# JasperSnoek/spearmint

Measured on AMD Instinct MI355X. Metric: EI candidate evaluations per second (N_cand x mcmc_iters / wall time), higher is better.
Workload: dtype f64; 1 GPU; C3: synthetic 32D, N_obs=2048, 200k candidates/GPU, mcmc_iters=20; N_obs=2048, candidates_per_gpu=200000, D=32, mcmc_iters=20, collective=torch.distributed all_gather_into_tensor

## Files before the change

### spearmint_amd/csrc/common.h

```cpp
#pragma once
#include <hip/hip_runtime.h>
#include <stdint.h>

typedef double d4 __attribute__((ext_vector_type(4)));
typedef double d2 __attribute__((ext_vector_type(2)));

#define MFMA_F64(a, b, c) __builtin_amdgcn_mfma_f64_16x16x4f64((a), (b), (c), 0, 0, 0)

#define SPX_NB 64
#define SPX_BM 128
#define SPX_BN 128
#define SPX_BK 16
#define SPX_PADN 128

#define SPX_COV_MATERN52 0
#define SPX_COV_MATERN32 1
#define SPX_COV_ARDSE 2

#define SPX_HT 4

static inline int64_t round_up(int64_t x, int64_t m) { return (x + m - 1) / m * m; }

void spx_note_attr_error(const char* kernel, size_t lds_bytes, hipError_t e);
#define SPX_LDS_ATTR(fn, bytes)                                                                                            \
    do {                                                                                                                   \
        hipError_t ae_ = hipFuncSetAttribute(reinterpret_cast<const void*>(fn), hipFuncAttributeMaxDynamicSharedMemorySize, \
                                             (int)(bytes));                                                                \
        if (ae_ != hipSuccess) spx_note_attr_error(#fn, (size_t)(bytes), ae_);                                             \
    } while (0)

void launch_scale_rows(hipStream_t s, const double* x, int64_t n, int64_t n_pad, int D, int Dp,
                       const double* ls , int ls_stride, int nh, double factor,
                       double* xs , double* sumsq ,
                       double* xs2 = nullptr ,
                       int* zero_ints = nullptr , int n_zero = 0);
void launch_lean_prologue(hipStream_t s, const double* x, int64_t n, int64_t n_pad, int D, int Dp, const double* ls,
                          int ls_stride, int nh, double* xs, double* sumsq, double* xs2, const double* vals,
                          const double* htab, double* rhs, int* info, int* flags, int64_t vals_stride = 0);
void launch_cov_self(hipStream_t s, const double* Xs, const double* s1, const double* X2s,
                     const double* htab, double* K, int N, int Np, int Dp, int nh, bool tiled = false,
                     int kind = SPX_COV_MATERN52);
void launch_cov_cross(hipStream_t s, const double* Xs, const double* s1, const double* Cs,
                      const double* s2, const double* htab, double* Kst, int N, int Np, int Mc,
                      int Dp, int nh, int kind = SPX_COV_MATERN52, int live_rows = 0 ,
                      bool allow_flat = true );
void launch_cross_mean(hipStream_t s, const double* Xs, const double* s1, const double* Cs,
                       const double* s2, const double* htab, const double* alpha, double* out,
                       int N, int Np, int Mc, int Dp, int nh, int kind = SPX_COV_MATERN52);
void launch_constraint_prob(hipStream_t s, const double* Xs, const double* s1, const double* Cs,
                            const double* s2, const double* htab, const double* alpha, double* out,
                            int N, int Np, int Mc, int Dp, int nh, int kind);
void launch_constraint_const(hipStream_t s, const double* htab, double* out, int Mc, int nh);

void launch_chol_diag(hipStream_t s, double* L, double* Dinv, int* info, int Np, int k, int nh, int updated = 0);
void launch_chol_panel(hipStream_t s, double* L, const double* Dinv, int Np, int k, int nh, double* rhs = nullptr);
void launch_lean_step(hipStream_t s, double* Lt, double* Dinv, int* info, double* rhs, double* diagL, int Np, int k,
                      int nh, int lazy);
void launch_lean_trsm(hipStream_t s, double* Lt, const double* Dinv, double* rhs, int Np, int k, int nh);
void launch_lean_step_ps(hipStream_t s, double* Lt, double* Dinv, int* info, double* rhs, double* diagL, int* flags,
                         int Np, int k, int nh);
struct FlowFused {
    const double* comp; const double* hyp; const double* vals; int D, hs;
    double* lp_out; int* info_out;
    int64_t vals_stride;
};
void launch_lean_flow(hipStream_t s, double* Lt, double* Dinv, int* info, double* rhs, double* diagL, int* lflags,
                      int* dflags, unsigned* tickets, int Np, int nh, int gen, bool alone,
                      const double* Xs, const double* X2s, const double* s1, const double* htab, int N, int Dp, int kind,
                      int* cu_busy, int spin_limit = 0, const FlowFused* fused = nullptr);
void launch_lean_rhs_init(hipStream_t s, const double* vals, const double* htab, double* rhs, int N, int Np, int nh,
                          int* info, int* flags, int64_t vals_stride = 0);
void launch_lean_logprob(hipStream_t s, const double* diagL, const double* rhs, const int* info, double* out, int* info_out,
                         int N, int Np, int nh);
void launch_trinv(hipStream_t s, const double* L, const double* Dinv, double* WT, int Np, int nh, bool tiled = false);
void launch_gamma(hipStream_t s, const double* WT, const double* vals, const double* htab,
                  double* gamma, int N, int Np, int nh);
void launch_gamma_multi(hipStream_t s, const double* WT_h, const double* rhs, const double* htab_h,
                        double* gamma, int N, int Np, int S);
// ... 57 lines not shown
```

### spearmint_amd/csrc/cov_kernels.hip

```cpp
#include "common.h"
#include "ei_device.h"

#ifndef SPX_COV_HOIST
#define SPX_COV_HOIST 1
#endif

#define SR_DC 32
template <int ROWS>
__device__ __forceinline__ void scale_rows_body(
    const double* __restrict__ x, int64_t n, int64_t n_pad, int D, int Dp,
    const double* __restrict__ ls, int ls_stride, double factor,
    double* __restrict__ xs, double* __restrict__ sumsq, double* __restrict__ xs2, int bx, int h)
{
#pragma clang fp contract(off)
    __shared__ double T[ROWS][SR_DC + 1];
    const int tid = threadIdx.x;
    const int64_t row0 = (int64_t)bx * ROWS;
    const int rows = (int)((n_pad - row0 < ROWS) ? (n_pad - row0) : ROWS);
    const int64_t row = row0 + tid;
    const double* lsh = ls + (size_t)h * ls_stride;
    double* o = xs + ((size_t)h * n_pad + row0) * Dp;
    double* o2 = xs2 ? xs2 + ((size_t)h * n_pad + row0) * Dp : nullptr;
    double acc = 0.0;
    for (int d0 = 0; d0 < Dp; d0 += SR_DC) {
// ... 246 lines not shown
    const double* __restrict__ Cs, const double* __restrict__ s2,
    const double* __restrict__ htab, const double* __restrict__ alpha,
    double* __restrict__ out, int N, int Np, int Mc, int Dp, int nchunks, int64_t ldo, int rows_per_wg, int live_rows)
{
    const int jtop = (MODE == 0 && live_rows > 0) ? live_rows : Np;
    const int jbeg = (MODE == 2 || MODE == 4) ? 0 : blockIdx.y * rows_per_wg;
    const int jend = (MODE == 2 || MODE == 4) ? Np : min(jtop, jbeg + rows_per_wg);
    cov_run<MODE, QC, KIND>(Xs, s1, Cs, s2, htab, alpha, out, N, Np, Mc, Dp, nchunks, ldo, blockIdx.z, blockIdx.x * 64, jbeg, jend);
}

template <int QC, int KIND>
__global__ __launch_bounds__(256, 2) void k_cov_flat(
    const double* __restrict__ Xs, const double* __restrict__ s1,
    const double* __restrict__ Cs, const double* __restrict__ s2,
    const double* __restrict__ htab, double* __restrict__ out, int N, int Np, int Mc, int Dp, int nchunks, int64_t ldo, int nh,
    int live_rows)
{
    const int jtop = live_rows > 0 ? live_rows : Np;
    const int nrc = (jtop + 127) >> 7, ncb = Mc >> 6;
    const int64_t per_h = (int64_t)ncb * nrc, U = per_h * nh;
    int64_t u = U * blockIdx.x / gridDim.x;
    const int64_t u1 = U * (blockIdx.x + 1) / gridDim.x;
    while (u < u1) {
        const int h = (int)(u / per_h);
        const int rem = (int)(u - (int64_t)h * per_h);
        const int cb = rem / nrc, rc = rem - cb * nrc;
        const int run = (int)min((int64_t)(nrc - rc), u1 - u);
        cov_run<0, QC, KIND>(Xs, s1, Cs, s2, htab, nullptr, out, N, Np, Mc, Dp, nchunks, ldo, h, cb * 64, rc * 128,
                             min(jtop, (rc + run) * 128));
        u += run;
    }
}

template <int MODE, int KIND>
static void launch_cov_kind(hipStream_t s, const double* Xs, const double* s1, const double* Cs,
                            const double* s2, const double* htab, const double* alpha, double* out,
                            int N, int Np, int Mc, int Dp, int nh, int64_t ldo, int live_rows, bool allow_flat)
{
    const int Q = Dp / 4;
    int rows_per_wg = (Np >= 1024) ? 512 : ((Np >= 256) ? 256 : 128);
#ifdef SPX_DEV_KNOBS
    static const char* rpw = getenv("SPX_COV_RPW");
    if (rpw && MODE == 3) rows_per_wg = atoi(rpw);
#endif
    const int row_top = (MODE == 0 && live_rows > 0) ? live_rows : Np;
    dim3 grid(Mc / 64, (MODE == 2 || MODE == 4) ? 1 : (row_top + rows_per_wg - 1) / rows_per_wg, nh);
    dim3 block(256);
    if (MODE == 0) {
        const int64_t places = 2 * (int64_t)spx_cov_cus(), wgs = (int64_t)grid.x * grid.y * grid.z;
        const int64_t units = (int64_t)nh * (Mc / 64) * (((live_rows > 0 ? live_rows : Np) + 127) / 128);
        if (wgs > places && units >= 4 * places && allow_flat) {
            const int64_t rounds = (units + 16 * places - 1) / (16 * places);
            const dim3 fgrid((unsigned)(places * rounds));
#define SPX_COVF_LAUNCH(QC_)                                                                                   \
    hipLaunchKernelGGL((k_cov_flat<QC_, KIND>), fgrid, block, 0, s, Xs, s1, Cs, s2, htab, out, N, Np, Mc, Dp, Q / QC_, ldo, nh, live_rows)
            if (Q == 1) SPX_COVF_LAUNCH(1);
            else if (Q == 2) SPX_COVF_LAUNCH(2);
            else if (Q == 4) SPX_COVF_LAUNCH(4);
            else SPX_COVF_LAUNCH(8);
#undef SPX_COVF_LAUNCH
            return;
        }
    }
#define SPX_COV_LAUNCH(QC_)                                                                        \
    hipLaunchKernelGGL((k_cov<MODE, QC_, KIND>), grid, block, 0, s, Xs, s1, Cs, s2, htab, alpha, out, N, \
                       Np, Mc, Dp, Q / QC_, ldo, rows_per_wg, live_rows)
// ... 60 lines not shown
```

### spearmint_amd/csrc/predict_kernels.hip

```cpp
#include "common.h"
#include "np_sum.h"
#include "ei_device.h"

#define BM SPX_BM
#define BN SPX_BN
#define BK SPX_BK
#define LDT 144

template <int NW, int STG, int ABL>
__global__ __launch_bounds__(64 * NW, NW / 2) void k_predict_gemm(
    const double* __restrict__ WT, const double* __restrict__ Kst,
    const double* __restrict__ gamma, double* __restrict__ part_ss,
    double* __restrict__ part_bg, int Np, int Mc, int nh, int ncb, int nrb,
    int part_nh , int part_h0 ,
    const double* __restrict__ gammaS , int S,
    double* __restrict__ part_bgS )
{
    extern __shared__ __attribute__((aligned(16))) double smem[];
    double* As = smem;
    double* Bs = smem + 2 * BK * LDT;

    const int tid = threadIdx.x;
    const int lane = tid & 63, wave = tid >> 6;
    const int g = lane >> 4, li = lane & 15;
// ... 241 lines not shown
    const int h = rem / ncbx;
    const int cb = (rem % ncbx) * 8 + xcd;
    if (cb >= ncb) return;

    const double* Ag = WT + (size_t)h * Np * Np + (size_t)ib * BM;
    const double* Bg = Kst + (size_t)h * Np * Mc + (size_t)cb * BN;
    const int nk = (ib + 1) * (BM / BK);
    typedef __attribute__((address_space(3))) void lds_void_t;
    const unsigned loff = (unsigned)lane * 16u;
    d4 acc[4][4];
#pragma unroll
    for (int mt = 0; mt < 4; ++mt)
#pragma unroll
        for (int nt = 0; nt < 4; ++nt) acc[mt][nt] = (d4){0.0, 0.0, 0.0, 0.0};

#define SPX_DMA_ROW(GPTR_, LPTR_)                                                                          \
    asm volatile("s_mov_b32 m0, %2\n\ts_nop 0\n\tglobal_load_lds_dwordx4 %0, %1"                          \
                 :: "v"(loff), "s"(GPTR_), "s"((unsigned)(size_t)(lds_void_t*)(LPTR_)) : "memory")
#define SPX_DMA_TILE(KT_, BUF_)                                                                            \
    {                                                                                                      \
        const size_t j0_ = (size_t)(KT_) * BK;                                                             \
        _Pragma("unroll") for (int q = 0; q < NQ; ++q) {                                                   \
            const int row = wave + NW * q;                                                                 \
            SPX_DMA_ROW(Ag + (j0_ + row) * Np, As + (BUF_) * BK * LDT + row * LDT);                        \
            SPX_DMA_ROW(Bg + (j0_ + row) * Mc, Bs + (BUF_) * BK * LDT + row * LDT);                        \
        }                                                                                                  \
    }
    SPX_DMA_TILE(0, 0)
    asm volatile("s_waitcnt vmcnt(0)" ::: "memory");
    __syncthreads();

    const int nfull = nk - BM / BK;
    int cur = 0;
    for (int j = 0; j < nk; ++j) {
        const int m0 = (j >= nfull) ? ((j - nfull - wm + 1) >> 1) : 0;
        if (j + 1 < nk) SPX_DMA_TILE(j + 1, cur ^ 1)
        const double* Ac = As + cur * BK * LDT + 16 * wm + li;
        const double* Bc = Bs + cur * BK * LDT + 64 * wn + li;
        if (m0 == 0) {
#pragma unroll
            for (int k0 = 0; k0 < BK; k0 += 4) {
                double a[4], b[4];
#pragma unroll
                for (int t = 0; t < 4; ++t) b[t] = Bc[(k0 + g) * LDT + 16 * t];
#pragma unroll
                for (int t = 0; t < 4; ++t) a[t] = Ac[(k0 + g) * LDT + 32 * t];
#pragma unroll
                for (int mt = 0; mt < 4; ++mt)
#pragma unroll
                    for (int nt = 0; nt < 4; ++nt) acc[mt][nt] = MFMA_F64(a[mt], b[nt], acc[mt][nt]);
            }
            asm volatile("s_waitcnt vmcnt(0)" ::: "memory");
            __syncthreads();
        } else {
#define SPX_TRI_G4(MT_)                                                      \
    _Pragma("unroll") for (int nt = 0; nt < 4; ++nt) acc[MT_][nt] = MFMA_F64(a[MT_], b[nt], acc[MT_][nt]);
#pragma unroll
            for (int k0 = 0; k0 < BK; k0 += 4) {
                double a[4], b[4];
#pragma unroll
                for (int t = 0; t < 4; ++t) b[t] = Bc[(k0 + g) * LDT + 16 * t];
#pragma unroll
                for (int t = 0; t < 4; ++t) a[t] = Ac[(k0 + g) * LDT + 32 * t];
                switch (m0) {
                    case 1: SPX_TRI_G4(1)
                    case 2: SPX_TRI_G4(2)
                    case 3: SPX_TRI_G4(3)
                    default: break;
                }
            }
#undef SPX_TRI_G4
            asm volatile("s_waitcnt vmcnt(0)" ::: "memory");
            __syncthreads();
        }
        cur ^= 1;
    }
#undef SPX_DMA_TILE
#undef SPX_DMA_ROW

    const double* gh = gamma + (size_t)h * Np + (size_t)ib * BM + 16 * wm;
    double gam[4][4];
#pragma unroll
    for (int mt = 0; mt < 4; ++mt)
#pragma unroll
        for (int r = 0; r < 4; ++r) gam[mt][r] = gh[32 * mt + g + 4 * r];
    double* red = smem;
#pragma unroll
    for (int nt = 0; nt < 4; ++nt) {
        double ss = 0.0, bg = 0.0;
#pragma unroll
        for (int mt = 0; mt < 4; ++mt)
#pragma unroll
            for (int r = 0; r < 4; ++r) {
                const double v = acc[mt][nt][r];
                ss = fma(v, v, ss);
                bg = fma(v, gam[mt][r], bg);
            }
        ss += __shfl_xor(ss, 16);
        bg += __shfl_xor(bg, 16);
        ss += __shfl_xor(ss, 32);
        bg += __shfl_xor(bg, 32);
        if (g == 0) {
            const int c = 64 * wn + 16 * nt + li;
            red[(wm * BN + c) * 2 + 0] = ss;
            red[(wm * BN + c) * 2 + 1] = bg;
        }
    }
// ... 500 lines not shown
```

### spearmint_amd/csrc/spx_api.hip

```cpp
#include <math.h>
#include <stdarg.h>
#include <stdio.h>
#include <string.h>

#include <algorithm>
#include <string>
#include <vector>

#include <chrono>

#include "spx_internal.h"
#include "np_sum.h"

#define SPX_VERSION 200

static const char* kStageNames[ST_COUNT] = {
    "scale_rows", "cov_self", "chol_diag", "chol_panel", "trinv", "gamma_alpha",
    "cov_cross", "cross_mean", "predict_gemm", "ei_finalize", "mean_argmax",
    "factor_total", "ei_run_total"};


std::string& spx_err_slot()
{
    static thread_local std::string g_err;
// ... 6 lines not shown
    return g_attr;
}

void spx_note_attr_error(const char* kernel, size_t lds_bytes, hipError_t e)
{
    char buf[384];
    snprintf(buf, sizeof buf, "hipFuncSetAttribute(%s, MaxDynamicSharedMemorySize = %zu) failed: %s", kernel, lds_bytes,
             hipGetErrorString(e));
    (void)hipGetLastError();
    if (spx_attr_err_slot().empty()) spx_attr_err_slot() = buf;
}

int spx_fail(int code, const char* fmt, ...)
{
    char buf[512];
    va_list ap;
    va_start(ap, fmt);
    vsnprintf(buf, sizeof buf, fmt, ap);
    va_end(ap);
    spx_err_slot() = buf;
    if (!spx_attr_err_slot().empty()) {
        spx_err_slot() += " [also: " + spx_attr_err_slot() + "]";
        spx_attr_err_slot().clear();
    }
    return code;
}

static int ensure_init(spx_handle* h)
{
    HIPCHK(hipSetDevice(h->device));
    if (!h->inited) {
        HIPCHK(hipStreamCreateWithFlags(&h->stream, hipStreamNonBlocking));
        HIPCHK(hipStreamCreateWithFlags(&h->stream2, hipStreamNonBlocking));
        for (int i = 0; i < 6; ++i) HIPCHK(hipEventCreateWithFlags(&h->ev_sync[i], hipEventDisableTiming));
        HIPCHK(hipEventCreate(&h->ev_t0));
        HIPCHK(hipEventCreate(&h->ev_t1));
        HIPCHK(hipEventCreateWithFlags(&h->ev_obs, hipEventDisableTiming));
        HIPCHK(hipEventCreateWithFlags(&h->ev_p0, hipEventDisableTiming));
        HIPCHK(hipEventCreateWithFlags(&h->ev_fac, hipEventDisableTiming));
        int ncu = 0;
        if (hipDeviceGetAttribute(&ncu, hipDeviceAttributeMultiprocessorCount, h->device) == hipSuccess && ncu > 0) h->n_cu = ncu;
        h->inited = true;
    }
    return SPX_OK;
}

static int ev_begin(spx_handle* h, int stage, hipStream_t strm)
{
    if (!h->timing) return -1;
    if (h->ev_used == h->ev_pool.size()) {
        spx_handle::Ev e;
        if (hipEventCreate(&e.a) != hipSuccess || hipEventCreate(&e.b) != hipSuccess) return -1;
        h->ev_pool.push_back(e);
    }
    spx_handle::Ev& e = h->ev_pool[h->ev_used];
    e.stage = stage;
    (void)hipEventRecord(e.a, strm);
    return (int)h->ev_used++;
}
static void ev_end(spx_handle* h, int id, hipStream_t strm)
{
    if (id >= 0) (void)hipEventRecord(h->ev_pool[id].b, strm);
}
static void ev_collect(spx_handle* h)
{
    for (size_t i = 0; i < h->ev_used; ++i) {
// ... 28 lines not shown
extern "C" {

int spx_version(void) { return SPX_VERSION; }
const char* spx_last_error(void) { return spx_err_slot().c_str(); }

int spx_device_count(void)
{
    int n = 0;
    hipError_t e = hipGetDeviceCount(&n);
    if (e != hipSuccess) return fail(SPX_ERR_HIP, "hipGetDeviceCount: %s", hipGetErrorString(e));
    return n;
}

int spx_create(int device_id, spx_handle** out)
{
    if (!out || device_id < 0) return fail(SPX_ERR_ARG, "spx_create: bad arguments");
    spx_handle* h = new spx_handle();
    h->device = device_id;
    *out = h;
    return SPX_OK;
}

void spx_destroy(spx_handle* h)
{
    if (!h) return;
    if (h->multi) { spx_multi_destroy(h->multi); delete h; return; }
    spx_comm_release(h);
    if (h->con) { spx_destroy(h->con); h->con = nullptr; }
    if (h->full) { spx_destroy(h->full); h->full = nullptr; }
    if (h->inited) {
        (void)hipSetDevice(h->device);
        (void)hipStreamSynchronize(h->stream);
        (void)hipStreamSynchronize(h->stream2);
        DevBuf* bufs[] = {&h->comp, &h->vals, &h->ldur, &h->cand, &h->hyp, &h->htab, &h->Xs, &h->X2s,
                          &h->s1, &h->Lm, &h->WT, &h->Dinv, &h->gamma, &h->alpha, &h->info, &h->lp,
                          &h->Cs[0], &h->s2[0], &h->Kst[0], &h->part_ss[0], &h->part_bg[0], &h->time_m[0],
                          &h->Cs[1], &h->s2[1], &h->Kst[1], &h->part_ss[1], &h->part_bg[1], &h->time_m[1],
                          &h->fantT, &h->gammaS, &h->bests, &h->part_bgS[0], &h->part_bgS[1],
                          &h->pt_x, &h->pt_k, &h->pt_dk, &h->pt_t, &h->pt_z, &h->pt_out, &h->pt_kt, &h->pt_dkt,
                          &h->ei_draw, &h->ei_mean, &h->mom_m, &h->mom_v, &h->mom_t, &h->am_val, &h->am_idx,
                          &h->am_out_val, &h->am_out_idx, &h->scratch, &h->sobol_dirs, &h->sobol_out, &h->rhs, &h->diagL, &h->ps_flags, &h->flow_flags,
                          &h->alphaS, &h->pt_u, &h->rec_send, &h->rec_recv, &h->rec_out, &h->ei_sum_full,
                          &h->con_tab, &h->con_Cs[0], &h->con_Cs[1], &h->con_s2[0], &h->con_s2[1], &h->con_p[0], &h->con_p[1],
                          &h->mom_c, &h->rhs_rows};
        for (DevBuf* b : bufs) b->release();
        h->pin_up.release();
        h->pin_res.release();
        h->pin_stage.release();
        for (auto& e : h->ev_pool) { (void)hipEventDestroy(e.a); (void)hipEventDestroy(e.b); }
        for (int i = 0; i < 6; ++i) (void)hipEventDestroy(h->ev_sync[i]);
        (void)hipEventDestroy(h->ev_t0);
        (void)hipEventDestroy(h->ev_t1);
        (void)hipEventDestroy(h->ev_obs);
        (void)hipEventDestroy(h->ev_p0);
        (void)hipEventDestroy(h->ev_fac);
        (void)hipStreamDestroy(h->stream);
        (void)hipStreamDestroy(h->stream2);
    }
    delete h;
}

int spx_set_option(spx_handle* h, const char* name, int64_t value)
{
    if (!h || !name) return fail(SPX_ERR_ARG, "spx_set_option: null");
    if (h->multi) return spx_multi_set_option(h->multi, name, value);
    if (!strcmp(name, "kstar_budget_bytes")) {
        h->kst_budget = value > 0 ? value : (512ll << 20);
        return SPX_OK;
    }
    if (!strcmp(name, "gemm_waves")) {
        if (!predict_gemm_variant_ok((int)value))
            return fail(SPX_ERR_ARG, "spx_set_option: gemm_waves=%lld is not a variant of this build", (long long)value);
        h->gemm_variant = (int)value;
        return SPX_OK;
    }
    if (!strcmp(name, "covar")) {
        if (value < SPX_COVAR_MATERN52 || value > SPX_COVAR_SE)
            return fail(SPX_ERR_ARG, "spx_set_option: covar=%lld is not one of SPX_COVAR_*", (long long)value);
        if (h->cov_kind != (int)value) { h->factored = false; h->ran = false; h->ran_time = false; h->S = 0; h->full_valid = false; }
        h->cov_kind = (int)value;
        return SPX_OK;
    }
    if (!strcmp(name, "lean_lazy")) {
        h->lean_lazy = value < 0 ? -1 : (value != 0);
        return SPX_OK;
    }
    if (!strcmp(name, "step_overlap")) {
        h->step_overlap = value < 0 ? -1 : (value != 0);
        return SPX_OK;
    }
// ... 21 lines not shown
        h->lean_flow = value < 0 ? -1 : (value != 0);
        h->flow_demoted = false;
        h->flow_clean = 0;
        return SPX_OK;
    }
    if (!strcmp(name, "flow_rearm_after")) {
        h->flow_rearm_after = value < 0 ? 16 : (int)std::min<int64_t>(value, 1 << 30);
        return SPX_OK;
    }
    if (!strcmp(name, "flow_spin_limit")) {
        h->flow_spin_limit = value <= 0 ? 0 : (int)std::min<int64_t>(value, 1 << 30);
        return SPX_OK;
    }
    if (!strcmp(name, "lean_ps")) {
        h->lean_ps = value < 0 ? -1 : (value != 0);
        return SPX_OK;
    }
    if (!strcmp(name, "lean_merge")) {
        h->lean_merge = value < 0 ? -1 : (value != 0);
        return SPX_OK;
    }
    if (!strcmp(name, "lean_one")) {
        h->lean_one = value < 0 ? -1 : (value != 0);
        return SPX_OK;
    }
    if (!strcmp(name, "lean_poll")) { h->lean_poll = value < 0 ? -1 : (value != 0); return SPX_OK; }
    if (!strcmp(name, "lean_zc")) { h->lean_zc = value < 0 ? -1 : (value != 0); return SPX_OK; }
    if (!strcmp(name, "stage_copies")) {
        h->stage_copies = value < 0 ? -1 : (value != 0);
        return SPX_OK;
    }
    if (!strcmp(name, "cov_flat")) {
        h->cov_flat = value < 0 ? -1 : (value != 0);
        return SPX_OK;
    }
    if (!strcmp(name, "gemm_partial")) {
        h->gemm_partial = value < 0 ? -1 : (value != 0);
        return SPX_OK;
    }
    if (!strcmp(name, "streams")) {
        h->nstreams = value == 2 ? 2 : 1;
        return SPX_OK;
    }
    if (!strcmp(name, "timing")) {
        h->timing = value != 0;
        memset(h->st_ms, 0, sizeof h->st_ms);
        memset(h->st_n, 0, sizeof h->st_n);
        return SPX_OK;
    }
    return fail(SPX_ERR_ARG, "spx_set_option: unknown option '%s'", name);
}

#define SPX_STAGE_MAX (8u << 20)
static void stage_begin(spx_handle* h) { h->stage_off = 0; }
static int stage_h2d(spx_handle* h, void* dst, const void* src, size_t bytes, hipStream_t s)
{
    if (h->stage_copies == 0 || bytes > SPX_STAGE_MAX || h->stage_off + bytes > 4 * (size_t)SPX_STAGE_MAX) {
        HIPCHK(hipMemcpyAsync(dst, src, bytes, hipMemcpyHostToDevice, s));
        return SPX_OK;
    }
    if (h->pin_stage.cap < h->stage_off + bytes) {
        if (h->stage_off) {
            HIPCHK(hipMemcpyAsync(dst, src, bytes, hipMemcpyHostToDevice, s));
            return SPX_OK;
        }
        int rc = h->pin_stage.reserve(bytes > (1u << 20) ? bytes : (1u << 20));
// ... 487 lines not shown
}

int spx_ei_step(spx_handle* h, int32_t flags)
{
    if (!h) return fail(SPX_ERR_ARG, "spx_ei_step: null handle");
    if (h->multi && (flags & SPX_FLAG_CONSTRAINED))
        return fail(SPX_ERR_ARG, "spx_ei_step: SPX_FLAG_CONSTRAINED is single-device only (multi-device handle)");
    if (h->multi) {
        int rc = spx_multi_factor(h->multi);
        return rc ? rc : spx_multi_ei_run(h->multi, flags & ~SPX_FLAG_TIME_ONLY);
    }
    if (h->timing || (flags & SPX_FLAG_TIMING) || !h->have_cand) {
        int rc = spx_factor(h);
        return rc ? rc : ei_run_impl(h, flags, false);
    }
    int rc = check_run_flags(h, flags, h->have_time ? 2 : 1);
    if (rc) return rc;
    if ((rc = factor_constraint(h))) return rc;
    h->handoff_timeout = false;
    rc = do_factor(h, false, false, true);
    if (rc) return rc;
    h->S = 0;
    rc = ei_run_impl(h, flags, true);
    if (rc == SPX_ERR_HIP && h->handoff_timeout && h->flow_used) {
        note_flow_timeout(h);
        rc = do_factor(h, false);
        if (!rc) rc = ei_run_impl(h, flags, false);
        if (!rc) warn_flow_fallback(h);
        return rc;
    }
    if (rc) {
        (void)hipStreamSynchronize(h->stream);
        (void)hipStreamSynchronize(h->stream2);
        (void)hipGetLastError();
        if (rc != SPX_ERR_NOT_PD) h->factored = false;
    }
    return rc;
}

static int ei_run_impl(spx_handle* h, int32_t flags, bool factor_pending)
{
    if (!h->factored && !factor_pending) return fail(SPX_ERR_ARG, "spx_ei_run: call spx_factor first");
    if (!h->have_cand) return fail(SPX_ERR_ARG, "spx_ei_run: no candidates set");
    const bool per_sec = (flags & SPX_FLAG_PER_SEC) != 0;
    const bool keep_mom = (flags & SPX_FLAG_KEEP_MOMENTS) != 0;
    const bool time_only = (flags & SPX_FLAG_TIME_ONLY) != 0;
    const bool constrained = (flags & SPX_FLAG_CONSTRAINED) != 0;
    int rc = check_run_flags(h, flags, h->nmodels);
    if (rc) return rc;
    if ((rc = ensure_init(h))) return rc;
    if (constrained && h->con_n > 0 && (!h->con_factored || h->con->cov_kind != h->cov_kind))
        return fail(SPX_ERR_ARG, "spx_ei_run: the constraint model is not factored (spx_factor after spx_set_constraint_model)");
    const int H = h->H, D = h->D, Dp = h->Dp, Np = h->Np, hs = 3 + D;
    const int64_t N = h->N, M = h->M, Mp = round_up(M, SPX_BN);
    const int nrb = Np / SPX_BM;
    int64_t Mc; int Hb;
    plan_chunks(h, &Mc, &Hb);
    const int S = h->S;
    if (S > 0) {
        if (h->fant_budget_S != S) {
            size_t mem_free = 0, mem_total = 0;
            int64_t b = 2048ll << 20;
            if (hipMemGetInfo(&mem_free, &mem_total) == hipSuccess) {
                const int64_t have = (int64_t)(mem_free / 8) + (int64_t)(h->part_bgS[0].cap + h->part_bgS[1].cap + h->scratch.cap) / 2;
                b = std::max<int64_t>(64ll << 20, std::min<int64_t>(b, have));
            } else (void)hipGetLastError();
            h->fant_budget = b;
            h->fant_budget_S = S;
        }
        const int64_t fant_budget = h->fant_budget;
        int64_t cap = fant_budget / ((int64_t)nrb * 2 * S * 8) / SPX_BN * SPX_BN;
        if (cap < SPX_BN) cap = SPX_BN;
        if (Mc > cap) {
            const int64_t nchunks = (Mp + cap - 1) / cap;
            Mc = round_up((Mp + nchunks - 1) / nchunks, SPX_BN);
        }
        int64_t hb = fant_budget / ((int64_t)nrb * 2 * S * 8 * Mc);
        if (hb > 65535 / S) hb = 65535 / S;
        if (hb < 1) hb = 1;
        if (hb < Hb) Hb = (int)hb;
    }

    const bool fused = Np == SPX_PADN && S == 0 && h->ei_fused != 0;
    h->last_fused = fused;
    const int ns = fused ? 1 : h->nstreams;
    for (int b = 0; b < 2; ++b) {
        if ((rc = h->Cs[b].reserve((size_t)H * Mc * Dp * 8))) return rc;
        if ((rc = h->s2[b].reserve((size_t)H * Mc * 8))) return rc;
        if (per_sec && (rc = h->time_m[b].reserve((size_t)H * Mc * 8))) return rc;
        if (constrained && (rc = h->con_p[b].reserve((size_t)H * Mc * 8))) return rc;
        if (constrained && h->con_n > 0 && (rc = h->con_Cs[b].reserve((size_t)H * Mc * Dp * 8))) return rc;
        if (constrained && h->con_n > 0 && (rc = h->con_s2[b].reserve((size_t)H * Mc * 8))) return rc;
        if (b < ns && !fused && !time_only) {
            if ((rc = h->Kst[b].reserve((size_t)Hb * Np * Mc * 8))) return rc;
            if (S > 0 && (rc = h->part_bgS[b].reserve((size_t)nrb * 2 * Hb * S * Mc * 8))) return rc;
        }
    }
    if (!fused && !time_only && (rc = h->part_ss[0].reserve((size_t)nrb * H * Mc * 8))) return rc;
    if (!fused && !time_only && (rc = h->part_bg[0].reserve((size_t)nrb * H * Mc * 8))) return rc;
    if (S > 0 && (rc = h->scratch.reserve((size_t)Hb * S * Mc * 8))) return rc;
    if ((rc = h->ei_draw.reserve((size_t)H * Mp * 8))) return rc;
    if ((rc = h->ei_mean.reserve((size_t)Mp * 8))) return rc;
    if (keep_mom) {
        if ((rc = h->mom_m.reserve((size_t)H * Mp * 8))) return rc;
        if ((rc = h->mom_v.reserve((size_t)H * Mp * 8))) return rc;
        if (per_sec && (rc = h->mom_t.reserve((size_t)H * Mp * 8))) return rc;
        if (constrained && (rc = h->mom_c.reserve((size_t)H * Mp * 8))) return rc;
    }
    const int nab = argmax_blocks(M);
    if ((rc = h->am_val.reserve((size_t)nab * 8))) return rc;
    if ((rc = h->am_idx.reserve((size_t)nab * 8))) return rc;
    if ((rc = h->am_out_val.reserve(8))) return rc;
    if ((rc = h->am_out_idx.reserve(8))) return rc;

    hipStream_t s = h->stream;
    if (flags & SPX_FLAG_TIMING) h->timing = true;
    h->ev_used = 0;
    hipEvent_t t0 = h->ev_t0, t1 = h->ev_t1;
    HIPCHK(hipEventRecord(t0, s));
    const int gemm_nlive = (!fused && h->gemm_partial != 0) ? predict_gemm_padding_plan(h->gemm_variant, (int)N, Np) : 0;
    const bool skip_pad = gemm_nlive > 0;
    const int cov_live_rows = 16 * gemm_nlive;
    h->last_skip_pad = skip_pad;

    const double* ls = h->hyp.d() + 3;
    const size_t nn = (size_t)Np * Np;
    hipStream_t G = h->stream, P = (ns == 2) ? h->stream2 : h->stream;
    const bool overlap = factor_pending && ns == 1 && h->step_overlap != 0;
    hipStream_t P0 = overlap ? h->stream2 : P;
    if (overlap) HIPCHK(hipStreamWaitEvent(P0, h->ev_obs, 0));
    if (factor_pending && ns == 2) HIPCHK(hipStreamWaitEvent(P, per_sec ? h->ev_fac : h->ev_obs, 0));
    int item = 0, chunk = 0;
    for (int64_t c0 = 0; c0 < Mp; c0 += Mc, ++chunk) {
        const int mc = (int)std::min<int64_t>(Mc, Mp - c0);
        const int64_t nreal = std::min<int64_t>(mc, M - c0);
        const double* xc = h->cand.d() + (size_t)c0 * D;
        const int par = chunk & 1;
        double* Cs = h->Cs[par].d();
        double* s2 = h->s2[par].d();
        double* tm = per_sec ? h->time_m[par].d() : nullptr;
        if (ns == 2 && chunk >= 2) HIPCHK(hipStreamWaitEvent(P, h->ev_sync[4 + par], 0));
        if (per_sec) {
            const bool side = overlap && chunk == 0;
            hipStream_t T = side ? G : P;
            double* CsT = side ? h->Cs[par ^ 1].d() : Cs;
            double* s2T = side ? h->s2[par ^ 1].d() : s2;
            TIMED_S(ST_SCALE, T, launch_scale_rows(T, xc, nreal, mc, D, Dp, ls + (size_t)H * hs, hs, H, 2.0, CsT, s2T));
            TIMED_S(ST_CROSS_MEAN, T, launch_cross_mean(T, h->Xs.d() + (size_t)H * Np * Dp, h->s1.d() + (size_t)H * Np, CsT, s2T,
                                                        h->htab.d() + (size_t)H * SPX_HT, h->alpha.d() + (size_t)H * Np, tm,
                                                        (int)N, Np, mc, Dp, H, dev_kind(h)));
            if (keep_mom)
                HIPCHK(hipMemcpy2DAsync(h->mom_t.d() + c0, (size_t)Mp * 8, tm, (size_t)mc * 8,
                                        (size_t)std::min<int64_t>(mc, Mp - c0) * 8, (size_t)H, hipMemcpyDeviceToDevice, T));
        }
        if (time_only) continue;
        double* cp = constrained ? h->con_p[par].d() : nullptr;
        if (constrained) {
            if (h->con_n > 0) {
                spx_handle* c = h->con;
                TIMED_S(ST_SCALE, P, launch_scale_rows(P, xc, nreal, mc, D, Dp, c->hyp.d() + 3, hs, H, 2.0, h->con_Cs[par].d(),
                                                       h->con_s2[par].d()));
                TIMED_S(ST_CROSS_MEAN, P, launch_constraint_prob(P, c->Xs.d(), c->s1.d(), h->con_Cs[par].d(), h->con_s2[par].d(),
                                                                 h->con_tab.d(), c->alpha.d(), cp, (int)c->N, c->Np, mc, Dp, H,
                                                                 dev_kind(h)));
            } else {
                TIMED_S(ST_CROSS_MEAN, P, launch_constraint_const(P, h->con_tab.d(), cp, mc, H));
            }
            if (keep_mom)
                HIPCHK(hipMemcpy2DAsync(h->mom_c.d() + c0, (size_t)Mp * 8, cp, (size_t)mc * 8,
                                        (size_t)std::min<int64_t>(mc, Mp - c0) * 8, (size_t)H, hipMemcpyDeviceToDevice, P));
        }
        hipStream_t Pc = (chunk == 0) ? P0 : P;
        TIMED_S(ST_SCALE, Pc, launch_scale_rows(Pc, xc, nreal, mc, D, Dp, ls, hs, H, 2.0, Cs, s2));
        if (fused && Pc != G) {
            HIPCHK(hipEventRecord(h->ev_p0, Pc));
            HIPCHK(hipStreamWaitEvent(G, h->ev_p0, 0));
        }
        if (fused)
            TIMED_S(ST_PREDICT_GEMM, G, launch_ei_fused128(G, dev_kind(h), h->WT.d(), h->gamma.d(), h->Xs.d(), h->s1.d(), Cs, s2,
                                                           h->htab.d(), tm, cp, h->best, h->ei_draw.d(), keep_mom ? h->mom_m.d() : nullptr,
                                                           keep_mom ? h->mom_v.d() : nullptr, (int)N, mc, Dp, H, c0, M, Mp, h->n_cu));
        for (int h0 = 0; h0 < (fused ? 0 : H); h0 += Hb, ++item) {
            const int nhb = std::min(Hb, H - h0);
            const int k = (ns == 2) ? (item & 1) : 0;
            if (ns == 2 && item >= 2) HIPCHK(hipStreamWaitEvent(P, h->ev_sync[2 + k], 0));
            hipStream_t Pi = (item == 0) ? Pc : P;
            TIMED_S(ST_COV_CROSS, Pi, launch_cov_cross(Pi, h->Xs.d() + (size_t)h0 * Np * Dp, h->s1.d() + (size_t)h0 * Np,
                                                      Cs + (size_t)h0 * mc * Dp, s2 + (size_t)h0 * mc,
                                                      h->htab.d() + (size_t)h0 * SPX_HT, h->Kst[k].d(), (int)N, Np, mc, Dp, nhb, dev_kind(h),
                                                      cov_live_rows, h->cov_flat != 0));
            if (ns == 2) {
                HIPCHK(hipEventRecord(h->ev_sync[k], P));
                HIPCHK(hipStreamWaitEvent(G, h->ev_sync[k], 0));
            } else if (Pi != G) {
                HIPCHK(hipEventRecord(h->ev_p0, Pi));
                HIPCHK(hipStreamWaitEvent(G, h->ev_p0, 0));
            }
            TIMED_S(ST_PREDICT_GEMM, G, launch_predict_gemm(G, h->gemm_variant, h->WT.d() + (size_t)h0 * nn, h->Kst[k].d(),
                                                            h->gamma.d() + (size_t)h0 * Np, h->part_ss[0].d(),
                                                            h->part_bg[0].d(), Np, mc, nhb, S > 0 ? nhb : H, S > 0 ? 0 : h0,
                                                            S > 0 ? h->gammaS.d() + (size_t)h0 * S * Np : nullptr, S,
                                                            S > 0 ? h->part_bgS[k].d() : nullptr, gemm_nlive));
            if (S > 0)
                TIMED_S(ST_EI_FINALIZE, G, launch_ei_finalize_fant(G, h->part_ss[0].d(), h->part_bgS[k].d(),
                                                                   h->htab.d() + (size_t)h0 * SPX_HT,
                                                                   h->bests.d() + (size_t)h0 * S,
                                                                   per_sec ? tm + (size_t)h0 * mc : nullptr,
                                                                   constrained ? cp + (size_t)h0 * mc : nullptr,
                                                                   h->ei_draw.d(), nrb, mc, nhb, S, c0, M, Mp, h0,
                                                                   h->scratch.d()));
            if (ns == 2) HIPCHK(hipEventRecord(h->ev_sync[2 + k], G));
        }
        if (S == 0 && !fused)
            TIMED_S(ST_EI_FINALIZE, G, launch_ei_finalize(G, h->part_ss[0].d(), h->part_bg[0].d(), h->htab.d(), tm, cp, h->best,
                                                          h->ei_draw.d(), keep_mom ? h->mom_m.d() : nullptr,
                                                          keep_mom ? h->mom_v.d() : nullptr, nrb, mc, H, c0, M, Mp, 0));
        if (ns == 2) HIPCHK(hipEventRecord(h->ev_sync[4 + par], G));
    }
    if (ns == 2 && (per_sec || constrained) && keep_mom) {
        HIPCHK(hipEventRecord(h->ev_sync[0], P));
        HIPCHK(hipStreamWaitEvent(G, h->ev_sync[0], 0));
    }
    const int n_info = factor_pending ? h->nmodels * H : 0;
// ... 572 lines not shown
    }
    std::vector<double> out((size_t)H * P * (1 + D));
    if ((rc = stage_d2h(h, out.data(), h->pt_out.p, out.size() * 8, s))) return rc;
    LAUNCHCHK();
    for (int p = 0; p < P; ++p) {
        double fsum = 0.0;
        double* g = grad + (size_t)p * D;
        for (int d = 0; d < D; ++d) g[d] = 0.0;
        for (int i = 0; i < H; ++i) {
            const double* o = &out[((size_t)i * P + p) * (1 + D)];
            fsum += -o[0];
            for (int d = 0; d < D; ++d) g[d] = g[d] + o[1 + d];
        }
        neg_cei[p] = fsum;
    }
    return SPX_OK;
}

int spx_get_stat(spx_handle* h, const char* name, int64_t* value)
{
    if (!h || !name || !value) return fail(SPX_ERR_ARG, "spx_get_stat: null");
    if (h->multi) {
        if (!strcmp(name, "ranks_seen") || !strcmp(name, "flow_fallbacks") || !strcmp(name, "flow_rearms") || !strcmp(name, "obs_dims"))
            return spx_multi_stat(h->multi, name, value);
        return fail(SPX_ERR_ARG, "spx_get_stat: ask the per-device handles (single-GPU handles only)");
    }
    if (!strcmp(name, "flow_fallbacks")) *value = h->flow_fallbacks;
    else if (!strcmp(name, "flow_enabled")) *value = (h->lean_flow != 0 && !h->flow_demoted);
    else if (!strcmp(name, "flow_rearms")) *value = h->flow_rearms;
    else if (!strcmp(name, "ranks_seen")) *value = h->comm ? h->ranks_seen : 1;
    else if (!strcmp(name, "n_cu")) *value = h->n_cu;
    else if (!strcmp(name, "obs_dims")) *value = h->have_obs ? h->D : 0;
    else if (!strcmp(name, "last_step_fused")) *value = h->last_fused ? 1 : 0;
    else if (!strcmp(name, "last_step_skipped_padding")) *value = h->last_skip_pad ? 1 : 0;
    else if (!strcmp(name, "hip_runtime_version") || !strcmp(name, "hip_driver_version")) {
        int v = 0;
        HIPCHK(name[4] == 'r' ? hipRuntimeGetVersion(&v) : hipDriverGetVersion(&v));
        *value = v;
    } else if (!strcmp(name, "clock_khz") || !strcmp(name, "mem_clock_khz") || !strcmp(name, "wall_clock_khz")
               || !strcmp(name, "l2_bytes") || !strcmp(name, "mem_bus_bits")) {
        int rc = ensure_init(h);
        if (rc) return rc;
        int v = 0;
        const hipDeviceAttribute_t a = !strcmp(name, "clock_khz") ? hipDeviceAttributeClockRate
            : !strcmp(name, "mem_clock_khz") ? hipDeviceAttributeMemoryClockRate
            : !strcmp(name, "wall_clock_khz") ? hipDeviceAttributeWallClockRate
            : !strcmp(name, "l2_bytes") ? hipDeviceAttributeL2CacheSize : hipDeviceAttributeMemoryBusWidth;
        HIPCHK(hipDeviceGetAttribute(&v, a, h->device));
        *value = v;
    }
    else return fail(SPX_ERR_ARG, "spx_get_stat: unknown statistic '%s'", name);
    return SPX_OK;
}

int spx_get_timings(spx_handle* h, double* ms, int64_t* launches, int n)
{
    if (!h) return fail(SPX_ERR_ARG, "null handle");
    if (h->multi) return spx_multi_get_timings(h->multi, ms, launches, n);
    for (int i = 0; i < n && i < ST_COUNT; ++i) {
        if (ms) ms[i] = h->st_ms[i];
        if (launches) launches[i] = h->st_n[i];
    }
    return ST_COUNT;
}

const char* spx_timing_name(int i) { return (i >= 0 && i < ST_COUNT) ? kStageNames[i] : ""; }
// ... 3 lines not shown
```

### spearmint_amd/csrc/spx_internal.h

```cpp
#pragma once
#include <stdarg.h>
#include <stdio.h>
#include <string.h>

#include <string>
#include <vector>

#include "../../include/spx.h"
#include "common.h"

std::string& spx_err_slot();
int spx_fail(int code, const char* fmt, ...);
#define fail spx_fail

#define HIPCHK(call)                                                                          \
    do {                                                                                      \
        hipError_t e_ = (call);                                                               \
        if (e_ != hipSuccess) {                                                               \
            (void)hipGetLastError();    \
            return fail(SPX_ERR_HIP, "%s failed: %s (%s:%d)", #call, hipGetErrorString(e_),   \
                        __FILE__, __LINE__);                                                  \
        }                                                                                     \
    } while (0)

// ... 32 lines not shown
    double* d() const { return (double*)p; }
};

struct PinBuf {
    void* p = nullptr;
    size_t cap = 0;
    int reserve(size_t bytes)
    {
        if (bytes <= cap) return SPX_OK;
        if (p) { (void)hipHostFree(p); p = nullptr; cap = 0; }
        if (bytes < 4096) bytes = 4096;
        hipError_t e = hipHostMalloc(&p, bytes, hipHostMallocCoherent);
        if (e != hipSuccess) {
            p = nullptr;
            (void)hipGetLastError();
            return fail(SPX_ERR_HIP, "hipHostMalloc(%zu bytes) failed: %s", bytes, hipGetErrorString(e));
        }
        cap = bytes;
        return SPX_OK;
    }
    void release() { if (p) (void)hipHostFree(p); p = nullptr; cap = 0; }
};

enum Stage {
    ST_SCALE = 0, ST_COV_SELF, ST_CHOL_DIAG, ST_CHOL_PANEL, ST_TRINV, ST_GAMMA_ALPHA,
    ST_COV_CROSS, ST_CROSS_MEAN, ST_PREDICT_GEMM, ST_EI_FINALIZE, ST_MEAN_ARGMAX,
    ST_FACTOR_TOTAL, ST_EI_RUN_TOTAL, ST_COUNT
};
struct spx_handle {
    int device = 0;
    bool inited = false;
    hipStream_t stream = nullptr;
    hipStream_t stream2 = nullptr;
    hipEvent_t ev_sync[6] = {nullptr, nullptr, nullptr, nullptr, nullptr, nullptr};
    hipEvent_t ev_t0 = nullptr, ev_t1 = nullptr;
    hipEvent_t ev_fac = nullptr;
    hipEvent_t ev_obs = nullptr, ev_p0 = nullptr;

    int64_t N = 0, M = 0, index_base = 0;
    int D = 0, Dp = 0, Np = 0, H = 0;
    bool have_obs = false, have_cand = false, have_hyp = false, have_time = false;
    bool factored = false, ran = false, ran_moments = false;
    bool ran_time = false;
    bool ran_tmean = false;
    int nmodels = 1;
    double best = 0.0;
    int not_pd_draw = -1, not_pd_pivot = -1;
    int64_t kst_budget = 512ll << 20;
    int nstreams = 1;
    int cov_kind = 0;
    int lean_lazy = -1;
    int gemm_variant = 0;
    int64_t fant_budget = 0;
    int fant_budget_S = -1;
    int lean_one = -1;
    int lean_poll = -1;
    int lean_zc = -1;
    double* fused_lp = nullptr;
    int* fused_info = nullptr;
    bool fused_ran = false;
    const void* info_clean_ptr = nullptr;
    size_t info_clean_bytes = 0;
    int cov_flat = -1;
    int gemm_partial = -1;
    bool last_skip_pad = false;
    struct spx_multi* multi = nullptr;
    struct spx_comm* comm = nullptr;

    std::vector<double> hyp_host, thyp_host;
    std::vector<double> up_raw, up_tab;

    DevBuf comp, vals, ldur, cand, hyp, htab;
    DevBuf Xs, X2s, s1, Lm, WT, Dinv, gamma, alpha, info, lp;
    DevBuf Cs[2], s2[2], Kst[2], part_ss[2], part_bg[2], time_m[2], ei_draw, ei_mean, mom_m, mom_v, mom_t;
    DevBuf am_val, am_idx, am_out_val, am_out_idx, scratch;
    int S = 0;
    DevBuf fantT, gammaS, bests, part_bgS[2];
    DevBuf alphaS;
    bool alphaS_valid = false;
    DevBuf pt_x, pt_k, pt_dk, pt_t, pt_z, pt_out, pt_kt, pt_dkt, pt_u;
    DevBuf rec_send, rec_recv, rec_out;
    int part_ph = 1;
    int64_t part_M = 0;
    int part_H = 0;
    bool ran_2d = false;
    DevBuf ei_sum_full;
    DevBuf sobol_dirs, sobol_out;
    spx_handle* con = nullptr;
    bool have_con = false, con_factored = false, ran_con = false;
    int64_t con_n = 0;
    std::vector<double> con_tab_host;
    DevBuf con_tab, con_Cs[2], con_s2[2], con_p[2], mom_c;
    spx_handle* full = nullptr;
    bool full_valid = false;
    std::vector<double> con_comp_host;
    DevBuf rhs_rows;
    bool rhs_rows_on = false;
    DevBuf rhs;
// ... 75 lines not shown
```

Measured before the change: 15.02 million EI evals/s.

## Double-buffer predict GEMM fragments and add opt-in covariance overlap on low-priority stream

Splits the predict GEMM K-loop into a full-tile loop that prefetches the next k-slice of A/B fragments from LDS while issuing MFMAs, and a separate triangular tail loop with per-row-tile guards. This aims to hide LDS latency behind MFMA work. It also adds a persistent slim cross-covariance kernel and a low-priority stream so covariance for the next item can overlap the GEMM. That overlap path is disabled by default and enabled through a new config knob. The prefetch raises register pressure, which could lower occupancy.

```diff
diff --git a/spearmint_amd/csrc/common.h b/spearmint_amd/csrc/common.h
--- a/spearmint_amd/csrc/common.h
+++ b/spearmint_amd/csrc/common.h
@@ -44,6 +44,8 @@
                       const double* s2, const double* htab, double* Kst, int N, int Np, int Mc,
                       int Dp, int nh, int kind = SPX_COV_MATERN52, int live_rows = 0 ,
                       bool allow_flat = true );
+void launch_cov_cross_slim(hipStream_t s, const double* Xs, const double* s1, const double* Cs, const double* s2,
+                           const double* htab, double* Kst, int N, int Np, int Mc, int Dp, int nh, int kind, int live_rows);
 void launch_cross_mean(hipStream_t s, const double* Xs, const double* s1, const double* Cs,
                        const double* s2, const double* htab, const double* alpha, double* out,
                        int N, int Np, int Mc, int Dp, int nh, int kind = SPX_COV_MATERN52);
diff --git a/spearmint_amd/csrc/cov_kernels.hip b/spearmint_amd/csrc/cov_kernels.hip
--- a/spearmint_amd/csrc/cov_kernels.hip
+++ b/spearmint_amd/csrc/cov_kernels.hip
@@ -302,6 +302,104 @@
     }
 }
 
+#define SPX_SLIM_VGPRS 72
+template <int QC, int KIND>
+__global__ __launch_bounds__(256, 7) void k_cov_slim(
+    const double* __restrict__ Xs, const double* __restrict__ s1,
+    const double* __restrict__ Cs, const double* __restrict__ s2,
+    const double* __restrict__ htab, double* __restrict__ out, int N, int Np, int Mc, int Dp, int nchunks, int64_t ldo, int nh,
+    int live_rows)
+{
+    const int lane = threadIdx.x & 63, wave = threadIdx.x >> 6;
+    const int g = lane >> 4, li = lane & 15;
+    const int Q = Dp >> 2;
+    const int jtop = live_rows > 0 ? live_rows : Np;
+    const int nrc = (jtop + 127) >> 7, ncb = Mc >> 6;
+    const int64_t per_h = (int64_t)ncb * nrc, U = per_h * nh;
+    int64_t u = U * blockIdx.x / gridDim.x;
+    const int64_t u1 = U * (blockIdx.x + 1) / gridDim.x;
+    while (u < u1) {
+        const int h = (int)(u / per_h);
+        const int rem = (int)(u - (int64_t)h * per_h);
+        const int cb = rem / nrc, rc = rem - cb * nrc;
+        const int run = (int)min((int64_t)(nrc - rc), u1 - u);
+        const int jbeg = rc * 128, jend = min(jtop, (rc + run) * 128);
+        const int c = cb * 64 + 16 * wave + li;
+        const double* Xh = Xs + (size_t)h * Np * Dp;
+        const double* pc = Cs + ((size_t)h * Mc + c) * Dp + g * Q;
+        const double* s1h = s1 + (size_t)h * Np;
+        const double amp2 = htab[h * SPX_HT + 2];
+        const double s2v = s2[(size_t)h * Mc + c];
+        double* oc = out + (size_t)h * Np * ldo + c;
+        double bf[QC];
+        if (nchunks == 1) {
+#pragma unroll
+            for (int q = 0; q < QC; ++q) bf[q] = pc[q];
+        }
+        for (int j0 = jbeg; j0 < jend; j0 += 16) {
+            d4 acc = (d4){0.0, 0.0, 0.0, 0.0};
+            for (int ch = 0; ch < nchunks; ++ch) {
+                double af[QC];
+                const double* pa = Xh + (size_t)(j0 + li) * Dp + g * Q + ch * QC;
+#pragma unroll
+                for (int q = 0; q < QC; ++q) af[q] = pa[q];
+                if (nchunks > 1) {
+#pragma unroll
+                    for (int q = 0; q < QC; ++q) bf[q] = pc[ch * QC + q];
+                }
+#pragma unroll
+                for (int q = 0; q < QC; ++q) acc = MFMA_F64(af[q], bf[q], acc);
+            }
+#pragma unroll
+            for (int r0 = 0; r0 < 4; r0 += 2) {
+#pragma clang fp contract(off)
+                double t[2], cv[2];
+#pragma unroll
+                for (int r = 0; r < 2; ++r) t[r] = (acc[r0 + r] - s1h[j0 + g + 4 * (r0 + r)]) - s2v;
+                corr_of_kind_t<KIND, 2>(t, cv);
+#pragma unroll
+                for (int r = 0; r < 2; ++r) {
+                    const int j = j0 + g + 4 * (r0 + r);
+                    const double amp_j = (j < N) ? amp2 : 0.0;
+                    oc[(size_t)j * ldo] = amp_j * cv[r];
+                }
+            }
+        }
+        u += run;
+    }
+}
+
+template <int KIND>
+static void launch_cov_slim_kind(hipStream_t s, const double* Xs, const double* s1, const double* Cs, const double* s2,
+                                 const double* htab, double* out, int N, int Np, int Mc, int Dp, int nh, int64_t ldo,
+                                 int live_rows, int max_wgs)
+{
+    const int Q = Dp / 4;
+    const int64_t units = (int64_t)nh * (Mc / 64) * (((live_rows > 0 ? live_rows : Np) + 127) / 128);
+    const dim3 grid((unsigned)std::max<int64_t>(1, std::min<int64_t>(units, max_wgs)));
+#define SPX_COVS_LAUNCH(QC_)                                                                                   \
+    hipLaunchKernelGGL((k_cov_slim<QC_, KIND>), grid, dim3(256), 0, s, Xs, s1, Cs, s2, htab, out, N, Np, Mc, Dp, Q / QC_, ldo, nh, live_rows)
+    if (Q == 1) SPX_COVS_LAUNCH(1);
+    else if (Q == 2) SPX_COVS_LAUNCH(2);
+    else if (Q == 4) SPX_COVS_LAUNCH(4);
+    else SPX_COVS_LAUNCH(8);
+#undef SPX_COVS_LAUNCH
+}
+
+int cov_slim_max_wgs() { return spx_cov_cus(); }
+
+void launch_cov_cross_slim(hipStream_t s, const double* Xs, const double* s1, const double* Cs, const double* s2,
+                           const double* htab, double* Kst, int N, int Np, int Mc, int Dp, int nh, int kind, int live_rows)
+{
+    const int wgs = cov_slim_max_wgs();
+    if (kind == SPX_COV_MATERN32)
+        launch_cov_slim_kind<SPX_COV_MATERN32>(s, Xs, s1, Cs, s2, htab, Kst, N, Np, Mc, Dp, nh, Mc, live_rows, wgs);
+    else if (kind == SPX_COV_ARDSE)
+        launch_cov_slim_kind<SPX_COV_ARDSE>(s, Xs, s1, Cs, s2, htab, Kst, N, Np, Mc, Dp, nh, Mc, live_rows, wgs);
+    else
+        launch_cov_slim_kind<SPX_COV_MATERN52>(s, Xs, s1, Cs, s2, htab, Kst, N, Np, Mc, Dp, nh, Mc, live_rows, wgs);
+}
+
 template <int MODE, int KIND>
 static void launch_cov_kind(hipStream_t s, const double* Xs, const double* s1, const double* Cs,
                             const double* s2, const double* htab, const double* alpha, double* out,
diff --git a/spearmint_amd/csrc/predict_kernels.hip b/spearmint_amd/csrc/predict_kernels.hip
--- a/spearmint_amd/csrc/predict_kernels.hip
+++ b/spearmint_amd/csrc/predict_kernels.hip
@@ -297,47 +297,57 @@
 
     const int nfull = nk - BM / BK;
     int cur = 0;
-    for (int j = 0; j < nk; ++j) {
-        const int m0 = (j >= nfull) ? ((j - nfull - wm + 1) >> 1) : 0;
-        if (j + 1 < nk) SPX_DMA_TILE(j + 1, cur ^ 1)
+    for (int j = 0; j < nfull; ++j) {
+        SPX_DMA_TILE(j + 1, cur ^ 1)
         const double* Ac = As + cur * BK * LDT + 16 * wm + li;
         const double* Bc = Bs + cur * BK * LDT + 64 * wn + li;
-        if (m0 == 0) {
+        double a[2][4], b[2][4];
+#pragma unroll
+        for (int t = 0; t < 4; ++t) b[0][t] = Bc[g * LDT + 16 * t];
+#pragma unroll
+        for (int t = 0; t < 4; ++t) a[0][t] = Ac[g * LDT + 32 * t];
+#pragma unroll
+        for (int kq = 0; kq < BK / 4; ++kq) {
+            const int c = kq & 1, n = c ^ 1;
+            if (kq + 1 < BK / 4) {
+#pragma unroll
+                for (int t = 0; t < 4; ++t) b[n][t] = Bc[(4 * (kq + 1) + g) * LDT + 16 * t];
+#pragma unroll
+                for (int t = 0; t < 4; ++t) a[n][t] = Ac[(4 * (kq + 1) + g) * LDT + 32 * t];
+            }
+#pragma unroll
+            for (int mt = 0; mt < 4; ++mt)
+#pragma unroll
+                for (int nt = 0; nt < 4; ++nt) acc[mt][nt] = MFMA_F64(a[c][mt], b[c][nt], acc[mt][nt]);
+            if (kq + 1 < BK / 4) __builtin_amdgcn_sched_barrier(0);
+        }
+        asm volatile("s_waitcnt vmcnt(0)" ::: "memory");
+        __syncthreads();
+        cur ^= 1;
+    }
+#pragma unroll 1
+    for (int d = 0; d < BM / BK; ++d) {
+        const int m0 = (d - wm + 1) >> 1;
+        if (d + 1 < BM / BK) SPX_DMA_TILE(nfull + d + 1, cur ^ 1)
+        const double* Ac = As + cur * BK * LDT + 16 * wm + li;
+        const double* Bc = Bs + cur * BK * LDT + 64 * wn + li;
+        if (m0 < 4) {
 #pragma unroll
             for (int k0 = 0; k0 < BK; k0 += 4) {
-                double a[4], b[4];
+                double b[4];
 #pragma unroll
                 for (int t = 0; t < 4; ++t) b[t] = Bc[(k0 + g) * LDT + 16 * t];
 #pragma unroll
-                for (int t = 0; t < 4; ++t) a[t] = Ac[(k0 + g) * LDT + 32 * t];
-#pragma unroll
                 for (int mt = 0; mt < 4; ++mt)
-#pragma unroll
-                    for (int nt = 0; nt < 4; ++nt) acc[mt][nt] = MFMA_F64(a[mt], b[nt], acc[mt][nt]);
-            }
-            asm volatile("s_waitcnt vmcnt(0)" ::: "memory");
-            __syncthreads();
-        } else {
-#define SPX_TRI_G4(MT_)                                                      \
-    _Pragma("unroll") for (int nt = 0; nt < 4; ++nt) acc[MT_][nt] = MFMA_F64(a[MT_], b[nt], acc[MT_][nt]);
-#pragma unroll
-            for (int k0 = 0; k0 < BK; k0 += 4) {
-                double a[4], b[4];
-#pragma unroll
-                for (int t = 0; t < 4; ++t) b[t] = Bc[(k0 + g) * LDT + 16 * t];
-#pragma unroll
-                for (int t = 0; t < 4; ++t) a[t] = Ac[(k0 + g) * LDT + 32 * t];
-                switch (m0) {
-                    case 1: SPX_TRI_G4(1)
-                    case 2: SPX_TRI_G4(2)
-                    case 3: SPX_TRI_G4(3)
-                    default: break;
-                }
-            }
-#undef SPX_TRI_G4
-            asm volatile("s_waitcnt vmcnt(0)" ::: "memory");
-            __syncthreads();
-        }
+                    if (mt >= m0) {
+                        const double a = Ac[(k0 + g) * LDT + 32 * mt];
+#pragma unroll
+                        for (int nt = 0; nt < 4; ++nt) acc[mt][nt] = MFMA_F64(a, b[nt], acc[mt][nt]);
+                    }
+            }
+        }
+        asm volatile("s_waitcnt vmcnt(0)" ::: "memory");
+        __syncthreads();
         cur ^= 1;
     }
 #undef SPX_DMA_TILE
diff --git a/spearmint_amd/csrc/spx_api.hip b/spearmint_amd/csrc/spx_api.hip
--- a/spearmint_amd/csrc/spx_api.hip
+++ b/spearmint_amd/csrc/spx_api.hip
@@ -62,6 +62,11 @@
     if (!h->inited) {
         HIPCHK(hipStreamCreateWithFlags(&h->stream, hipStreamNonBlocking));
         HIPCHK(hipStreamCreateWithFlags(&h->stream2, hipStreamNonBlocking));
+        {
+            int prio_least = 0, prio_greatest = 0;
+            HIPCHK(hipDeviceGetStreamPriorityRange(&prio_least, &prio_greatest));
+            HIPCHK(hipStreamCreateWithPriority(&h->stream_lo, hipStreamNonBlocking, prio_least));
+        }
         for (int i = 0; i < 6; ++i) HIPCHK(hipEventCreateWithFlags(&h->ev_sync[i], hipEventDisableTiming));
         HIPCHK(hipEventCreate(&h->ev_t0));
         HIPCHK(hipEventCreate(&h->ev_t1));
@@ -156,6 +161,7 @@
         (void)hipSetDevice(h->device);
         (void)hipStreamSynchronize(h->stream);
         (void)hipStreamSynchronize(h->stream2);
+        if (h->stream_lo) (void)hipStreamSynchronize(h->stream_lo);
         DevBuf* bufs[] = {&h->comp, &h->vals, &h->ldur, &h->cand, &h->hyp, &h->htab, &h->Xs, &h->X2s,
                           &h->s1, &h->Lm, &h->WT, &h->Dinv, &h->gamma, &h->alpha, &h->info, &h->lp,
                           &h->Cs[0], &h->s2[0], &h->Kst[0], &h->part_ss[0], &h->part_bg[0], &h->time_m[0],
@@ -180,6 +186,7 @@
         (void)hipEventDestroy(h->ev_fac);
         (void)hipStreamDestroy(h->stream);
         (void)hipStreamDestroy(h->stream2);
+        if (h->stream_lo) (void)hipStreamDestroy(h->stream_lo);
     }
     delete h;
 }
@@ -267,6 +274,14 @@
     }
     if (!strcmp(name, "cov_flat")) {
         h->cov_flat = value < 0 ? -1 : (value != 0);
+        return SPX_OK;
+    }
+    if (!strcmp(name, "cov_overlap")) {
+        h->cov_overlap = value < 0 ? SPX_COV_OVERLAP_DEFAULT : (value == 2 ? 2 : (value != 0));
+        return SPX_OK;
+    }
+    if (!strcmp(name, "cov_overlap_min_np")) {
+        h->cov_overlap_min_np = value < 0 ? 1024 : (int)std::min<int64_t>(value, 1 << 30);
         return SPX_OK;
     }
     if (!strcmp(name, "gemm_partial")) {
@@ -820,6 +835,7 @@
     if (rc) {
         (void)hipStreamSynchronize(h->stream);
         (void)hipStreamSynchronize(h->stream2);
+        if (h->stream_lo) (void)hipStreamSynchronize(h->stream_lo);
         (void)hipGetLastError();
         if (rc != SPX_ERR_NOT_PD) h->factored = false;
     }
@@ -871,7 +887,11 @@
 
     const bool fused = Np == SPX_PADN && S == 0 && h->ei_fused != 0;
     h->last_fused = fused;
-    const int ns = fused ? 1 : h->nstreams;
+    const int64_t n_items = ((Mp + Mc - 1) / Mc) * ((H + Hb - 1) / Hb);
+    const bool cov_ov = !fused && !time_only && h->cov_overlap == 1 && h->nstreams == 1 && n_items >= 2 && Np >= h->cov_overlap_min_np;
+    h->last_overlap = cov_ov;
+    const int ns = fused ? 1 : (cov_ov ? 2 : h->nstreams);
+    const bool slim = cov_ov || (h->cov_overlap == 2 && !fused);
     for (int b = 0; b < 2; ++b) {
         if ((rc = h->Cs[b].reserve((size_t)H * Mc * Dp * 8))) return rc;
         if ((rc = h->s2[b].reserve((size_t)H * Mc * 8))) return rc;
@@ -913,7 +933,7 @@
 
     const double* ls = h->hyp.d() + 3;
     const size_t nn = (size_t)Np * Np;
-    hipStream_t G = h->stream, P = (ns == 2) ? h->stream2 : h->stream;
+    hipStream_t G = h->stream, P = cov_ov ? h->stream_lo : ((ns == 2) ? h->stream2 : h->stream);
     const bool overlap = factor_pending && ns == 1 && h->step_overlap != 0;
     hipStream_t P0 = overlap ? h->stream2 : P;
     if (overlap) HIPCHK(hipStreamWaitEvent(P0, h->ev_obs, 0));
@@ -973,10 +993,16 @@
             const int k = (ns == 2) ? (item & 1) : 0;
             if (ns == 2 && item >= 2) HIPCHK(hipStreamWaitEvent(P, h->ev_sync[2 + k], 0));
             hipStream_t Pi = (item == 0) ? Pc : P;
-            TIMED_S(ST_COV_CROSS, Pi, launch_cov_cross(Pi, h->Xs.d() + (size_t)h0 * Np * Dp, h->s1.d() + (size_t)h0 * Np,
-                                                      Cs + (size_t)h0 * mc * Dp, s2 + (size_t)h0 * mc,
-                                                      h->htab.d() + (size_t)h0 * SPX_HT, h->Kst[k].d(), (int)N, Np, mc, Dp, nhb, dev_kind(h),
-                                                      cov_live_rows, h->cov_flat != 0));
+            if (slim)
+                TIMED_S(ST_COV_CROSS, Pi, launch_cov_cross_slim(Pi, h->Xs.d() + (size_t)h0 * Np * Dp, h->s1.d() + (size_t)h0 * Np,
+                                                               Cs + (size_t)h0 * mc * Dp, s2 + (size_t)h0 * mc,
+                                                               h->htab.d() + (size_t)h0 * SPX_HT, h->Kst[k].d(), (int)N, Np, mc, Dp, nhb,
+                                                               dev_kind(h), cov_live_rows));
+            else
+                TIMED_S(ST_COV_CROSS, Pi, launch_cov_cross(Pi, h->Xs.d() + (size_t)h0 * Np * Dp, h->s1.d() + (size_t)h0 * Np,
+                                                          Cs + (size_t)h0 * mc * Dp, s2 + (size_t)h0 * mc,
+                                                          h->htab.d() + (size_t)h0 * SPX_HT, h->Kst[k].d(), (int)N, Np, mc, Dp, nhb, dev_kind(h),
+                                                          cov_live_rows, h->cov_flat != 0));
             if (ns == 2) {
                 HIPCHK(hipEventRecord(h->ev_sync[k], P));
                 HIPCHK(hipStreamWaitEvent(G, h->ev_sync[k], 0));
@@ -1615,6 +1641,7 @@
     else if (!strcmp(name, "n_cu")) *value = h->n_cu;
     else if (!strcmp(name, "obs_dims")) *value = h->have_obs ? h->D : 0;
     else if (!strcmp(name, "last_step_fused")) *value = h->last_fused ? 1 : 0;
+    else if (!strcmp(name, "last_overlap")) *value = h->last_overlap ? 1 : 0;
     else if (!strcmp(name, "last_step_skipped_padding")) *value = h->last_skip_pad ? 1 : 0;
     else if (!strcmp(name, "hip_runtime_version") || !strcmp(name, "hip_driver_version")) {
         int v = 0;
diff --git a/spearmint_amd/csrc/spx_internal.h b/spearmint_amd/csrc/spx_internal.h
--- a/spearmint_amd/csrc/spx_internal.h
+++ b/spearmint_amd/csrc/spx_internal.h
@@ -88,6 +88,7 @@
     bool inited = false;
     hipStream_t stream = nullptr;
     hipStream_t stream2 = nullptr;
+    hipStream_t stream_lo = nullptr;
     hipEvent_t ev_sync[6] = {nullptr, nullptr, nullptr, nullptr, nullptr, nullptr};
     hipEvent_t ev_t0 = nullptr, ev_t1 = nullptr;
     hipEvent_t ev_fac = nullptr;
@@ -120,6 +121,10 @@
     int cov_flat = -1;
     int gemm_partial = -1;
     bool last_skip_pad = false;
+#define SPX_COV_OVERLAP_DEFAULT 0
+    int cov_overlap = SPX_COV_OVERLAP_DEFAULT;
+    int cov_overlap_min_np = 1024;
+    bool last_overlap = false;
     struct spx_multi* multi = nullptr;
     struct spx_comm* comm = nullptr;
 
```

After: 15.09 million EI evals/s, median of 6. Within noise of the previous version (+0.5%).
